# BUBLET/uav-airvision

Measured on AMD Instinct MI355X. Metric: stereo frames/sec (LK+stereo+MSCKF-update) at 752x480, higher is better.
Workload: dtype u8/int32 windows, f32 normal equations

## Files before the change

uav_airvision_amd/csrc/msckf.hip:

```cpp
#include <math.h>

#include <memory>
#include <new>
#include <vector>

#include "av_common.h"

namespace {

constexpr int IMU_DIM = 21;

#ifndef AV_FILTER_WAVE_PRIO
#define AV_FILTER_WAVE_PRIO 3
#endif
#define AV_FILTER_PRIO() __builtin_amdgcn_s_setprio(AV_FILTER_WAVE_PRIO)

__device__ __forceinline__ double av_rsqrt_f64(double d)
{
    const bool tiny = d < 1e-280;
    const double ds = tiny ? d * 0x1p200 : d;
    double y = __builtin_amdgcn_rsq(ds);
    const double h = 0.5 * ds;
    y = y * (1.5 - h * y * y);
    y = y * (1.5 - h * y * y);
// ... 772 lines not shown
        for (int r = 0; r < 3; ++r) sv[r] = u[r] / uu;
    } else if (tid == R2) {
        double dv[3] = {a.v_null[0] - a.v_new[0], a.v_null[1] - a.v_new[1], a.v_null[2] - a.v_new[2]};
        double dp[3] = {a.dt * a.v_null[0] + a.p_null[0] - a.p_new[0], a.dt * a.v_null[1] + a.p_null[1] - a.p_new[1], a.dt * a.v_null[2] + a.p_null[2] - a.p_new[2]};
        const double* g = a.gravity;
        w1[0] = -dv[2] * g[1] + dv[1] * g[2]; w1[1] = dv[2] * g[0] - dv[0] * g[2]; w1[2] = -dv[1] * g[0] + dv[0] * g[1];
        w2[0] = -dp[2] * g[1] + dp[1] * g[2]; w2[1] = dp[2] * g[0] - dp[0] * g[2]; w2[2] = -dp[1] * g[0] + dp[0] * g[1];
    }
    __syncthreads();
    __shared__ unsigned frow[IMU_DIM], fcol[IMU_DIM], prow[IMU_DIM];
    for (int i = tid; i < N * N; i += NT) F[i] *= a.dt;
    if (tid >= R2 && tid < R2 + N) {
        const int r = tid - R2; unsigned m = 0;
        for (int k = 0; k < N; ++k) if (F[r * N + k] != 0.0) m |= 1u << k;
        frow[r] = m;
    } else if (tid >= R3 && tid < R3 + N) {
        const int c = tid - R3; unsigned m = 0;
        for (int k = 0; k < N; ++k) if (F[k * N + c] != 0.0) m |= 1u << k;
        fcol[c] = m;
    }
    __syncthreads();
    for (int i = tid; i < N * N; i += NT) {
        int r = i / N, c = i - r * N; double s = 0;
        for (unsigned m = frow[r]; m; m &= m - 1) { const int k = __builtin_ctz(m); s += F[r * N + k] * F[k * N + c]; }
        F2[i] = s;
    }
    __syncthreads();
    for (int i = tid; i < N * N; i += NT) {
        int r = i / N, c = i - r * N; double s = 0;
        for (unsigned m = fcol[c]; m; m &= m - 1) { const int k = __builtin_ctz(m); s += F2[r * N + k] * F[k * N + c]; }
        Phi[i] = (r == c ? 1.0 : 0.0) + F[i] + F2[i] / 2. + s / 6.;
    }
    __syncthreads();
    if (tid < 9) {
        int r = tid / 3, c = tid % 3; double s = 0;
        for (int k = 0; k < 3; ++k) s += Rnew[r * 3 + k] * Rnull[c * 3 + k];
        Phi[r * N + c] = s;
    } else if (tid >= R1 && tid < R1 + 6) {
        const int t6 = tid - R1, blk = t6 / 3, r = t6 % 3;
        const int row = (blk == 0 ? 6 : 12) + r;
        const double* wv = blk == 0 ? w1 : w2;
        const double p0 = Phi[row * N], p1 = Phi[row * N + 1], p2 = Phi[row * N + 2];
        const double Au = p0 * u[0] + p1 * u[1] + p2 * u[2];
        const double d = Au - wv[r];
        Phi[row * N] = p0 - d * sv[0]; Phi[row * N + 1] = p1 - d * sv[1]; Phi[row * N + 2] = p2 - d * sv[2];
    } else if (tid >= R2 && tid < R2 + N) {
        const int r = tid - R2; unsigned m = 0;
        for (int k = 0; k < N; ++k) if (Phi[r * N + k] != 0.0) m |= 1u << k;
        if (r < 3 || (r >= 6 && r < 9) || (r >= 12 && r < 15)) m |= 7u;
        prow[r] = m;
    }
    __syncthreads();
    for (int i = tid; i < N * 12; i += NT) {
        int r = i / 12, c = i - r * 12; double s = 0;
        for (unsigned m = prow[r]; m; m &= m - 1) { const int k = __builtin_ctz(m); s += Phi[r * N + k] * G[k * 12 + c]; }
        T[i] = s;
    }
    for (int i = tid; i < N * N; i += NT) {
        int r = i / N, c = i - r * N; double s = 0;
        if (P11s) { for (unsigned m = prow[r]; m; m &= m - 1) { const int k = __builtin_ctz(m); s += Phi[r * N + k] * P11s[k * N + c]; } }
        else      { for (unsigned m = prow[r]; m; m &= m - 1) { const int k = __builtin_ctz(m); s += Phi[r * N + k] * a.P[(size_t)k * a.ld + c]; } }
        F2[i] = s;
        if (P11s) {
            double s2 = 0;
            for (unsigned m = prow[r]; m; m &= m - 1) { const int k = __builtin_ctz(m); s2 += Phi[r * N + k] * PhiT[k * N + c]; }
            Q[i] = s2;
        }
    }
    __syncthreads();
    for (int i = tid; i < N * N; i += NT) {
        int r = i / N, c = i - r * N; double s = 0, q = 0;
        for (int k = 0; k < 12; ++k) q += T[r * 12 + k] * a.noise[k / 3] * T[c * 12 + k];
        q = q * a.dt;
        for (unsigned m = prow[c]; m; m &= m - 1) { const int k = __builtin_ctz(m); s += F2[r * N + k] * Phi[c * N + k]; }
        F[i] = s + q;
    }
    __syncthreads();
    if (P11s) {
        for (int i = tid; i < N * N; i += NT) {
            int r = i / N, c = i - r * N;
            PhiT[i] = Q[i];
            P11s[i] = (F[r * N + c] + F[c * N + r]) / 2.;
        }
        __syncthreads();
        return;
    }
    const int nc = a.n - N;
    for (int c0 = 0; c0 < nc; c0 += N) {
        const int w = min(N, nc - c0);
        for (int i = tid; i < N * w; i += NT) {
            int r = i / w, c = i - r * w; double s = 0;
            for (unsigned m = prow[r]; m; m &= m - 1) { const int k = __builtin_ctz(m); s += Phi[r * N + k] * a.P[(size_t)k * a.ld + N + c0 + c]; }
            T[i] = s;
        }
        __syncthreads();
        for (int i = tid; i < N * w; i += NT) {
            int r = i / w, c = i - r * w;
            a.P[(size_t)r * a.ld + N + c0 + c] = T[i];
            a.P[(size_t)(N + c0 + c) * a.ld + r] = T[i];
        }
        __syncthreads();
    }
    for (int i = tid; i < N * N; i += NT) {
        int r = i / N, c = i - r * N;
        a.P[(size_t)r * a.ld + c] = (F[r * N + c] + F[c * N + r]) / 2.;
    }
}

__global__ __launch_bounds__(256) void propagate_kernel(PropArgs a) { propagate_body(a); }

struct AugArgs { double* P; int n, ld; double R_ic[9]; double sk[9]; };

template <int NT = 256>
__device__ __forceinline__ void augment_body(const AugArgs& a)
{
    __shared__ double J[6 * IMU_DIM];
    __shared__ double C[36];
    const int tid = threadIdx.x, N = IMU_DIM, n = a.n;
    for (int i = tid; i < 6 * N; i += NT) J[i] = 0.0;
    __syncthreads();
    if (tid < 9) {
        int r = tid / 3, c = tid % 3;
        J[r * N + c] = a.R_ic[tid];
        J[r * N + 15 + c] = r == c ? 1.0 : 0.0;
        J[(3 + r) * N + c] = a.sk[tid];
        J[(3 + r) * N + 12 + c] = r == c ? 1.0 : 0.0;
        J[(3 + r) * N + 18 + c] = r == c ? 1.0 : 0.0;
    }
    __syncthreads();
    for (int i = tid; i < 6 * n; i += NT) {
        int r = i / n, c = i - r * n; double s = 0;
        for (int k = 0; k < N; ++k) s += J[r * N + k] * a.P[(size_t)k * a.ld + c];
        a.P[(size_t)(n + r) * a.ld + c] = s;
    }
    __syncthreads();
    if (tid < 36) {
        int r = tid / 6, c = tid % 6; double s = 0;
        for (int k = 0; k < N; ++k) s += a.P[(size_t)(n + r) * a.ld + k] * J[c * N + k];
        C[tid] = s;
    }
    __syncthreads();
    for (int i = tid; i < 6 * n; i += NT) {
        int r = i / n, c = i - r * n;
        a.P[(size_t)c * a.ld + n + r] = a.P[(size_t)(n + r) * a.ld + c];
    }
    if (tid < 36) {
        int r = tid / 6, c = tid % 6;
        a.P[(size_t)(n + r) * a.ld + n + c] = (C[r * 6 + c] + C[c * 6 + r]) / 2.;
    }
}

__global__ __launch_bounds__(256) void augment_kernel(AugArgs a) { augment_body(a); }

__device__ __forceinline__ void remove_cam_body(double* P, double* scratch, int n, int ld, int start)
{
    const int tid = threadIdx.x, m = n - 6;
    for (int i = tid; i < m * m; i += (int)blockDim.x) {
        int r = i / m, c = i - r * m;
        int sr = r < start ? r : r + 6, sc = c < start ? c : c + 6;
        scratch[i] = P[(size_t)sr * ld + sc];
    }
    __syncthreads();
    for (int i = tid; i < m * m; i += (int)blockDim.x) {
        int r = i / m, c = i - r * m;
        P[(size_t)r * ld + c] = scratch[i];
    }
}
__device__ __forceinline__ void remove_two_cams_body(double* P, double* scratch, int n, int ld, int s0, int s1)
{
    const int tid = threadIdx.x, m = n - 12;
    for (int i = tid; i < m * m; i += (int)blockDim.x) {
        const int r = i / m, c = i - r * m;
        if (r < s0 && c < s0) continue;
        const int sr = r < s0 ? r : (r + 6 < s1 ? r + 6 : r + 12), sc = c < s0 ? c : (c + 6 < s1 ? c + 6 : c + 12);
        scratch[i] = P[(size_t)sr * ld + sc];
    }
    __syncthreads();
    for (int i = tid; i < m * m; i += (int)blockDim.x) {
        const int r = i / m, c = i - r * m;
        if (r < s0 && c < s0) continue;
        P[(size_t)r * ld + c] = scratch[i];
    }
}
__global__ __launch_bounds__(256) void remove_cam_kernel(double* P, double* scratch, int n, int ld, int start) { remove_cam_body(P, scratch, n, ld, start); }

struct UpdArgs {
    double* P; int n, ld;
    const double* Hsrc; const double* rsrc;
    const int* blk_row; const int* blk_len; int n_blk;
    double* W;
    int ldt;
    const int* cols; int nc;
    unsigned long long* prof;
    double* T;
    double* Kt;
    double* Pn;
    double* dx;
    double obs_noise;
    int m;
    double* Sbuf;
    int mode;
    int kdir;
    int round;
    int hld;
    int* status;
};
constexpr int UPD_BAD_PIVOT = -2;

template <typename T> using av_gptr = T __attribute__((address_space(1)))*;
struct UpdArgsG {
    av_gptr<double> P; int n, ld;
    av_gptr<const double> Hsrc; av_gptr<const double> rsrc;
    av_gptr<const int> blk_row; av_gptr<const int> blk_len; int n_blk;
    av_gptr<double> W; int ldt;
    av_gptr<const int> cols; int nc;
    av_gptr<unsigned long long> prof;
    av_gptr<double> T; av_gptr<double> Kt; av_gptr<double> Pn; av_gptr<double> dx;
    double obs_noise; int m;
    av_gptr<double> Sbuf;
    int mode, kdir, round, hld;
    av_gptr<int> status;
};
__device__ __forceinline__ UpdArgsG upd_load(const UpdArgs* __restrict__ arr, int i)
{
    const UpdArgs a = arr[i];
    UpdArgsG g;
    g.P = (av_gptr<double>)a.P; g.n = a.n; g.ld = a.ld; g.Hsrc = (av_gptr<const double>)a.Hsrc; g.rsrc = (av_gptr<const double>)a.rsrc;
    g.blk_row = (av_gptr<const int>)a.blk_row; g.blk_len = (av_gptr<const int>)a.blk_len; g.n_blk = a.n_blk;
    g.W = (av_gptr<double>)a.W; g.ldt = a.ldt; g.cols = (av_gptr<const int>)a.cols; g.nc = a.nc; g.prof = (av_gptr<unsigned long long>)a.prof;
    g.T = (av_gptr<double>)a.T; g.Kt = (av_gptr<double>)a.Kt; g.Pn = (av_gptr<double>)a.Pn; g.dx = (av_gptr<double>)a.dx;
    g.obs_noise = a.obs_noise; g.m = a.m; g.Sbuf = (av_gptr<double>)a.Sbuf; g.mode = a.mode; g.kdir = a.kdir; g.round = a.round; g.hld = a.hld;
    g.status = (av_gptr<int>)a.status;
    return g;
}

constexpr int UT = 1024;

__host__ __device__ inline bool upd_compress(int m, int nc) { return m > nc && (2 * m > 3 * nc || m > 136); }
__host__ __device__ inline int upd_k(int m, int nc) { return upd_compress(m, nc) ? nc : m; }

__device__ __forceinline__ double block_sum(double v, double* red)
{
    const int tid = threadIdx.x;
    v = wave_sum_f64(v);
    __syncthreads();
    if ((tid & 63) == 0) red[tid >> 6] = v;
    __syncthreads();
    double s = 0;
#pragma unroll
    for (int i = 0; i < UT / 64; ++i) s += red[i];
    return s;
}


__device__ __forceinline__ void reflector_scalars(double nrm2, double ajj, double& alpha, double& v0, double& tau)
{
    double r = nrm2 > 0 ? __builtin_amdgcn_rsq(nrm2) : 0.0;
    r = r * (1.5 - 0.5 * nrm2 * r * r);
    r = r * (1.5 - 0.5 * nrm2 * r * r);
    const double nrm = nrm2 * r;
    alpha = ajj >= 0 ? -nrm : nrm;
    v0 = ajj - alpha;
    const double vtv = nrm2 - 2 * alpha * ajj + alpha * alpha;
    double t = vtv > 0 ? __builtin_amdgcn_rcp(vtv) : 0.0;
    t = t * (2.0 - vtv * t);
    t = t * (2.0 - vtv * t);
    tau = 2.0 * t;
}

template <int CPW, int RPL>
__device__ __forceinline__ void qr_in_registers(const UpdArgs& a, int m, int nc, const int* srcrow, double* vb0, double* vb1, double* qsc,
                                                double* Wt, size_t ldt, double* rcol)
{
    const int tid = threadIdx.x, wave = tid >> 6, lane = tid & 63;
    double x[CPW][RPL];
#pragma unroll
    for (int l = 0; l < CPW; ++l) {
        const int c = wave + 16 * l;
#pragma unroll
        for (int t = 0; t < RPL; ++t) {
            const int row = lane + 64 * t;
            double v = 0.0;
            if (row < m && c <= nc) v = c < nc ? a.Hsrc[(size_t)srcrow[row] * a.ld + a.cols[c]] : a.rsrc[srcrow[row]];
            x[l][t] = v;
        }
    }
    __syncthreads();
    if (a.prof && tid == 0) a.prof[1] = __builtin_amdgcn_s_memrealtime();
    for (int j = 0; j < nc; ++j) {
        double* vb = (j & 1) ? vb1 : vb0;
        double* sc = qsc + 2 * (j & 1);
        if (wave == (j & 15)) {
            const int lj = j >> 4, tj = j >> 6;
            double part = 0, cand = 0;
#pragma unroll
            for (int l = 0; l < CPW; ++l) if (l == lj) {
#pragma unroll
                for (int t = 0; t < RPL; ++t) {
                    const int row = lane + 64 * t;
                    if (row >= j) part += x[l][t] * x[l][t];
                    if (t == tj) cand = x[l][t];
                }
            }
            const double nrm2 = wave_sum_f64(part);
            const double ajj = __shfl(cand, j & 63, 64);
            double alpha, v0o, tauo;
// ... 1053 lines not shown
```

uav_airvision_amd/csrc/msckf_dev.inc:

```

namespace {

constexpr int DEV_BUCKETS = 2;
constexpr int DEV_IMU_BATCH = 16;
constexpr int DEV_LDS_KEYS = 2048;

enum { DFAIL_NONE = 0, DFAIL_CAMS = 1, DFAIL_FRAMES = 2, DFAIL_STACK = 3, DFAIL_PIVOT = 4, DFAIL_TABLE = 5, DFAIL_OBS = 6, DFAIL_ROWS = 7 };

struct DState {
    double ts;
    double q[4], p[3], v[3], bg[3], ba[3];
    double R_ic[9], t_ci[3];
    double qn[4], pn[3], vn[3];
    double gravity[3];
    double tracking_rate;
    long long next_imu_id;
    int n, ncam;
    int active;
    int failed;
    int first_img, null_aliased;
    int prune, rm0, rm1;
    int n_prune_steps;
    int n_two_pass;
    int resets;
// ... 115 lines not shown
    for (int i = 0; i < 4; ++i) S.q[i] = qo[i];
    for (int i = 0; i < 3; ++i) {
        S.bg[i] += dx[3 + i]; S.v[i] += dx[6 + i]; S.ba[i] += dx[9 + i]; S.p[i] += dx[12 + i];
        if (S.null_aliased) { S.vn[i] += dx[6 + i]; S.pn[i] += dx[12 + i]; }
    }
    double de[4], Re[9], Rn[9];
    h_small_angle(dx + 15, de); h_to_rotation(de, Re);
    for (int r = 0; r < 3; ++r) for (int c = 0; c < 3; ++c) Rn[r * 3 + c] = Re[r * 3] * S.R_ic[c] + Re[r * 3 + 1] * S.R_ic[3 + c] + Re[r * 3 + 2] * S.R_ic[6 + c];
    for (int i = 0; i < 9; ++i) S.R_ic[i] = Rn[i];
    for (int i = 0; i < 3; ++i) S.t_ci[i] += dx[18 + i];
}
__device__ void dev_inject_cam(double* cq, double* cp, const double* d)
{
    double q4[4], co[4];
    h_small_angle(d, q4); h_quat_mul(q4, cq, co);
    for (int i = 0; i < 4; ++i) cq[i] = co[i];
    for (int i = 0; i < 3; ++i) cp[i] += d[3 + i];
}
__device__ void dev_apply_update(const DevArgs& a, int s, DState* D)
{
    const int st = a.stacked[s];
    if (threadIdx.x == 0) {
        if (st == UPD_BAD_PIVOT) D->failed = DFAIL_PIVOT;
        else if (st < 0) D->failed = DFAIL_STACK;
        else if (st > 0) { DState L = *D; dev_inject_imu(L, a.dx + (size_t)s * a.ld); *D = L; }
    }
    if (st > 0 && (int)threadIdx.x < D->ncam) {
        const size_t c = (size_t)s * a.cs + threadIdx.x;
        dev_inject_cam(a.cam_q + 4 * c, a.cam_p + 3 * c, a.dx + (size_t)s * a.ld + IMU_DIM + 6 * threadIdx.x);
    }
    __syncthreads();
}

__global__ __launch_bounds__(64) void dk_state(DevArgs a)
{
    AV_FILTER_PRIO();
    const int s = blockIdx.x * 64 + threadIdx.x;
    if (blockIdx.x == 0 && threadIdx.x < 16) a.cnt_next[threadIdx.x] = 0;
    if (s >= a.S) return;
    DState* Dg = a.st + s;
    const DCtl C = a.ctl[s];
    {
        DState L = *Dg;
        DState* D = &L;
        DCov cv; cv.act = 0; cv.cnt = 0; cv.first = C.imu_first; cv.pad = 0;
        if (C.has_init) {
            for (int i = 0; i < 4; ++i) D->q[i] = C.q0[i];
            for (int i = 0; i < 3; ++i) { D->bg[i] = C.bg0[i]; D->gravity[i] = C.g0[i]; }
        }
        int act = C.active && !D->failed;
        if (act && D->ncam + 1 > a.cs) { D->failed = DFAIL_CAMS; act = 0; }
        if (act && D->first_img) { D->first_img = 0; D->ts = C.t_frame; }
        D->active = act; D->prune = 0;
        if (act) {
            double* P = a.P + (size_t)s * a.pstride;
            const int n = D->n, ld = a.ld;
            for (int k = 0; k < C.imu_cnt; ++k) {
                PropArgs pa;
                const DImu m = a.imu[C.imu_first + k];
                pa.P = P; pa.n = n; pa.ld = ld; pa.dt = m.t - D->ts;
                for (int i = 0; i < 3; ++i) { pa.gyro[i] = m.w[i] - D->bg[i]; pa.acc[i] = m.a[i] - D->ba[i]; pa.gravity[i] = D->gravity[i]; }
                for (int i = 0; i < 4; ++i) { pa.q_old[i] = D->q[i]; pa.noise[i] = a.noise[i]; }
                dev_predict_new_state(*D, pa.dt, pa.gyro, pa.acc);
                for (int i = 0; i < 4; ++i) { pa.q_new[i] = D->q[i]; pa.q_null[i] = D->qn[i]; }
                for (int i = 0; i < 3; ++i) { pa.v_null[i] = D->vn[i]; pa.p_null[i] = D->pn[i]; pa.v_new[i] = D->v[i]; pa.p_new[i] = D->p[i]; }
                for (int i = 0; i < 4; ++i) D->qn[i] = D->q[i];
                for (int i = 0; i < 3; ++i) { D->pn[i] = D->p[i]; D->vn[i] = D->v[i]; }
                D->null_aliased = 1;
                D->ts = m.t;
                a.prop[C.imu_first + k] = pa;
            }
            double Rwi[9], Rwc[9], tw[3], cq[4];
            h_to_rotation(D->q, Rwi);
            for (int r = 0; r < 3; ++r) for (int c = 0; c < 3; ++c) Rwc[r * 3 + c] = D->R_ic[r * 3] * Rwi[c] + D->R_ic[r * 3 + 1] * Rwi[3 + c] + D->R_ic[r * 3 + 2] * Rwi[6 + c];
            h_mtv(Rwi, D->t_ci, tw);
            h_to_quaternion(Rwc, cq);
            const size_t c = (size_t)s * a.cs + D->ncam;
            a.cam_id[c] = D->next_imu_id++;
            for (int i = 0; i < 4; ++i) { a.cam_q[4 * c + i] = cq[i]; a.cam_qn[4 * c + i] = cq[i]; }
            for (int i = 0; i < 3; ++i) a.cam_p[3 * c + i] = D->p[i] + tw[i];
            cv.act = 1; cv.cnt = C.imu_cnt;
            cv.aa.P = P; cv.aa.n = n; cv.aa.ld = ld;
            for (int i = 0; i < 9; ++i) cv.aa.R_ic[i] = D->R_ic[i];
            const double sk[9] = {0, -tw[2], tw[1], tw[2], 0, -tw[0], -tw[1], tw[0], 0};
            for (int i = 0; i < 9; ++i) cv.aa.sk[i] = sk[i];
            D->n = n + 6; D->ncam += 1;
            a.ncam[s] = D->ncam; a.nstate[s] = D->n;
            for (int i = 0; i < 3; ++i) a.grav[3 * s + i] = D->gravity[i];
        }
        a.cov[s] = cv;
        *Dg = L;
    }
}

struct DImuState { double t, p[3], q[4], v[3], w[3]; };
static_assert(sizeof(DImuState) == 112, "av_imu_state is 112 bytes");
struct IrOut { DImuState* rec; int* n; int cap; };
__global__ __launch_bounds__(64) void dk_imu_rate(DevArgs a, IrOut R)
{
    AV_FILTER_PRIO();
    const int s = blockIdx.x, lane = threadIdx.x;
    const DCov cv = a.cov[s];
    const int had = cv.act ? cv.cnt : 0, wr = had < R.cap ? had : R.cap, k0 = had - wr;
    if (lane == 0) { R.n[2 * (size_t)s] = had; R.n[2 * (size_t)s + 1] = wr; }
    constexpr int W = (int)(sizeof(DImuState) / 8);
    double* out = reinterpret_cast<double*>(R.rec + (size_t)s * R.cap);
    for (int e = lane; e < wr * W; e += 64) {
        const int j = e / W, f = e - j * W;
        const size_t i = (size_t)cv.first + k0 + j;
        const PropArgs& pa = a.prop[i];
        out[e] = f == 0 ? a.imu[i].t : (f < 4 ? pa.p_new[f - 1] : (f < 8 ? pa.q_new[f - 4] : (f < 11 ? pa.v_new[f - 8] : pa.gyro[f - 11])));
    }
}

template <int NT>
__global__ __launch_bounds__(NT) void dk_cov(DevArgs a)
{
    AV_FILTER_PRIO();
    __shared__ double P11s[IMU_DIM * IMU_DIM], PhiT[IMU_DIM * IMU_DIM], work[PROP_LDS_DOUBLES];
    const int s = blockIdx.x, tid = threadIdx.x, N = IMU_DIM;
    const DCov cv = a.cov[s];
    if (!cv.act) return;
    double* P = cv.aa.P;
    const int n = cv.aa.n, ld = cv.aa.ld;
    auto stamp = [&](int i) { if (a.prof && s == 0 && tid == 0) a.prof[i] = __builtin_amdgcn_s_memrealtime(); };
    stamp(0);
    if (cv.cnt > 0) {
        for (int i = tid; i < N * N; i += NT) { const int r = i / N, c = i - r * N; P11s[i] = P[(size_t)r * ld + c]; PhiT[i] = r == c ? 1.0 : 0.0; }
        __syncthreads();
        for (int k = 0; k < cv.cnt; ++k) propagate_body<true, NT>(a.prop[cv.first + k], P11s, PhiT, work);
        stamp(1);
        const int nc = n - N;
        constexpr int CW = 64, NRQ = NT / CW;
        const int cl = tid % CW, rq = tid / CW;
        for (int c0 = 0; c0 < nc; c0 += CW) {
            const int c = c0 + cl;
            const bool in = c < nc;
            __syncthreads();
            for (int k = rq; k < IMU_DIM; k += NRQ) work[k * CW + cl] = in ? P[(size_t)k * ld + N + c] : 0.0;
            __syncthreads();
#pragma unroll 1
            for (int r = rq; r < IMU_DIM; r += NRQ) {
                double sum = 0;
#pragma unroll 7
                for (int k = 0; k < IMU_DIM; ++k) sum += PhiT[r * N + k] * work[k * CW + cl];
                if (in) { P[(size_t)r * ld + N + c] = sum; P[(size_t)(N + c) * ld + r] = sum; }
            }
        }
        for (int i = tid; i < N * N; i += NT) { const int r = i / N, c = i - r * N; P[(size_t)r * ld + c] = P11s[i]; }
        __syncthreads();
    }
    stamp(2);
    augment_body<NT>(cv.aa);
}

__device__ void dev_build_candidates(const DevArgs& a, const AvsTeam& T, const AvsStore& V, int s, int nc, const int* cand, bool full,
                                     int i0, int i1, const int* e0, const int* e1, int ph, int* lb )
{
    const int tid = threadIdx.x;
    const size_t f0 = (size_t)s * a.FS, ob = (size_t)s * a.obs_stride;
    if (tid < 8) lb[tid] = 0;
    __syncthreads();
    int obs_run = 0, row_run = 0, tobs_run = 0;
    for (int base = 0; base < nc; base += (int)blockDim.x) {
        const int k = base + tid;
        const bool in = k < nc;
        const int fs = in ? cand[k] : 0;
        const int nall = in ? V.m_nobs[fs] : 0;
        const int nobs = full ? nall : (in ? 2 : 0);
        const int init = in ? V.m_init[fs] : 1;
        int to, tr, tt;
        const int o = obs_run + T.excl_scan(nobs, &to);
        const int r = row_run + T.excl_scan(in ? 4 * nobs - 3 : 0, &tr);
        const int t = tobs_run + T.excl_scan((!full && !init) ? nall : 0, &tt);
        if (in) {
            const size_t f = f0 + k;
            a.f_off[f] = (int)(ob + o); a.f_rowoff[f] = r; a.f_dof[f] = full ? nobs - 1 : 2; a.f_mslot[f] = fs;
            if (!full) a.t_off[f] = (int)(ob + t);
            if (full) (void)avs_collect(V, fs, a.obs_cam + ob + o, a.obs_z + 4 * (ob + o));
            else {
                a.obs_cam[ob + o] = i0; a.obs_cam[ob + o + 1] = i1;
                const double* z0 = V.fr_z + ((size_t)avs_lslot(e0[k]) * V.cap + avs_lidx(e0[k])) * 4;
                const double* z1 = V.fr_z + ((size_t)avs_lslot(e1[k]) * V.cap + avs_lidx(e1[k])) * 4;
                for (int e = 0; e < 4; ++e) { a.obs_z[4 * (ob + o) + e] = z0[e]; a.obs_z[4 * (ob + o + 1) + e] = z1[e]; }
            }
            int valid = 1, tri = 0;
            if (init) { for (int e = 0; e < 3; ++e) a.f_pos[3 * f + e] = V.m_pos[(size_t)3 * fs + e]; }
            else {
                valid = 0; tri = 1;
                int* tc = full ? a.obs_cam + ob + o : a.t_obs_cam + ob + t;
                double* tz = full ? a.obs_z + 4 * (ob + o) : a.t_obs_z + 4 * (ob + t);
                if (!full) (void)avs_collect(V, fs, tc, tz);
                if (a.trans_thr >= 0) {
                    const size_t ca = (size_t)s * a.cs + tc[0], cb = (size_t)s * a.cs + tc[nall - 1];
                    double Ra[9], d[3] = {tz[0], tz[1], 1.0}, dw[3];
                    const double nd = h_norm3(d); d[0] /= nd; d[1] /= nd; d[2] /= nd;
                    h_to_rotation(a.cam_q + 4 * ca, Ra); h_mtv(Ra, d, dw);
                    const double tv[3] = {a.cam_p[3 * cb] - a.cam_p[3 * ca], a.cam_p[3 * cb + 1] - a.cam_p[3 * ca + 1], a.cam_p[3 * cb + 2] - a.cam_p[3 * ca + 2]};
                    const double par = tv[0] * dw[0] + tv[1] * dw[1] + tv[2] * dw[2];
                    const double o3[3] = {tv[0] - par * dw[0], tv[1] - par * dw[1], tv[2] - par * dw[2]};
                    if (!(h_norm3(o3) > a.trans_thr)) tri = 0;
                }
            }
            a.f_valid[f] = valid;
            const int bk = (full && nobs > 8) ? 1 : 0;
            V.tmp_a[k] = (bk << 24) | atomicAdd(&lb[bk], 1);
            V.tmp_b[k] = tri ? atomicAdd(&lb[5], 1) : -1;
        }
        obs_run += to; row_run += tr; tobs_run += tt;
    }
    __syncthreads();
    if (tid == 0) {
        a.f_off[f0 + nc] = (int)(ob + obs_run);
        if (!full) a.t_off[f0 + nc] = (int)(ob + tobs_run);
        a.n_cand[s] = nc;
        int shift = 0;
        if (row_run > a.rows_cap) {
            const int base = ph == 0 ? atomicAdd(&a.cnt[8 * ph + 4], row_run) : -1;
            if (base >= 0 && base + row_run <= a.pool_rows) shift = (a.S - s) * a.rows_cap + base;
            else shift = -1;
        }
        lb[6] = shift;
        a.over[s] = 0;
        if (shift < 0) { DState* D = a.st + s; D->failed = DFAIL_ROWS; D->active = 0; a.n_cand[s] = 0; }
    }
    __syncthreads();
    const int shift = lb[6];
    if (shift < 0) {
        for (int k = tid; k < nc; k += (int)blockDim.x) { a.f_rowoff[f0 + k] = -1; a.f_valid[f0 + k] = 0; V.tmp_b[k] = -1; }
        __syncthreads();
        return;
    }
    if (tid < 6) { const int c = lb[tid]; lb[tid] = c > 0 ? atomicAdd(&a.cnt[8 * ph + tid], c) : 0; }
    __syncthreads();
    const size_t lstride = (size_t)a.S * a.cap;
    for (int k = tid; k < nc; k += (int)blockDim.x) {
        const size_t f = f0 + k;
        const int v = V.tmp_a[k], bk = v >> 24;
        a.blist[bk * lstride + lb[bk] + (v & 0xFFFFFF)] = (int)f;
        if (V.tmp_b[k] >= 0) a.tlist[lb[5] + V.tmp_b[k]] = (int)f;
        if (shift > 0) a.f_rowoff[f] += shift;
    }
    __syncthreads();
}

__device__ __forceinline__ void dk_append_body(const DevArgs& a, unsigned long long* lds_keys)
{
    __shared__ int red[8], lb[8];
    const int s = blockIdx.x, tid = threadIdx.x;
    DState* D = a.st + s;
    if (!D->active) { if (tid == 0) { a.n_cand[s] = 0; a.over[s] = 0; a.f_off[(size_t)s * a.FS] = 0; } return; }
    AvsTeam T; T.red = red;
    AvsStore V = dev_store(a, s);
    if (a.cap <= DEV_LDS_KEYS) V.keys = lds_keys;
    const int before = V.hdr[AVS_LIVE];
    __syncthreads();
    auto stamp = [&](int i) { if (a.prof && s == 0 && tid == 0) a.prof[i] = __builtin_amdgcn_s_memrealtime(); };
    stamp(3);
    int tracked = 0;
    const int nk = a.msg_n[s] < a.msg_cap ? a.msg_n[s] : a.msg_cap;
    const int slot = avs_add_frame(T, V, a.msg_ids + (size_t)s * a.msg_cap, a.msg_uv + (size_t)s * a.msg_cap * 4, nk, &tracked);
    if (slot < 0) {
        if (tid == 0) { D->failed = slot == -1 ? DFAIL_FRAMES : DFAIL_TABLE; D->active = 0; a.n_cand[s] = 0; a.over[s] = 0; }
        return;
    }
    if (tid == 0) D->tracking_rate = tracked / ((double)before + 1e-5);
    int* cand = a.cand + (size_t)s * a.cap; int* inval = a.e0 + (size_t)s * a.cap;
    int nc = 0, ni = 0;
    stamp(4);
    avs_select_lost(T, V, cand, &nc, inval, &ni);
    stamp(5);
    dev_build_candidates(a, T, V, s, nc, cand, true, 0, 0, nullptr, nullptr, 0, lb);
    stamp(6);
    dev_triangulate_own(a, V, s, nc, false);
    stamp(7);
    if (tid == 0 && lb[6] > 0) D->n_two_pass += 1;
    avs_erase(T, V, cand, nc);
    avs_erase(T, V, inval, ni);
    stamp(8);
}

__device__ __forceinline__ void dk_begin_body(const DevArgs& a)
{
    AV_FILTER_PRIO();
    __shared__ unsigned long long keys8[DEV_LDS_KEYS];
    dk_append_body(a, keys8);
}
__global__ __launch_bounds__(256, 5) void dk_begin4(DevArgs a) { dk_begin_body(a); }

__device__ void dev_find_redundant(const DevArgs& a, int s, const DState& D, int* r0, int* r1)
{
    const int nc = D.ncam, key = nc - 4;
    const size_t c0 = (size_t)s * a.cs;
    int idx = key + 1, firstc = 0;
    double Rk[9];
    h_to_rotation(a.cam_q + 4 * (c0 + key), Rk);
    int sel[2];
    for (int k = 0; k < 2; ++k) {
        double Rc[9], RR[9], qq[4];
        h_to_rotation(a.cam_q + 4 * (c0 + idx), Rc);
        for (int r = 0; r < 3; ++r) for (int c = 0; c < 3; ++c) RR[r * 3 + c] = Rc[r * 3] * Rk[c * 3] + Rc[r * 3 + 1] * Rk[c * 3 + 1] + Rc[r * 3 + 2] * Rk[c * 3 + 2];
        h_to_quaternion(RR, qq);
        const double d[3] = {a.cam_p[3 * (c0 + idx)] - a.cam_p[3 * (c0 + key)], a.cam_p[3 * (c0 + idx) + 1] - a.cam_p[3 * (c0 + key) + 1], a.cam_p[3 * (c0 + idx) + 2] - a.cam_p[3 * (c0 + key) + 2]};
        const double ang = 2 * acos(qq[3]);
        if (ang < 0.2618 && h_norm3(d) < 0.4 && D.tracking_rate > 0.5) sel[k] = idx;
        else { sel[k] = firstc; ++firstc; }
// ... 542 lines not shown
```

Before: 233,000.

## Specialize covariance kernel for 64-thread blocks with sparsity-masked propagation chains

Adds a dk_cov<64> specialization that runs IMU covariance propagation, cross-covariance update and state augmentation with a single wavefront. It uses per-row and per-column nonzero bitmasks of F and Phi to skip zero terms in the matrix products, and keeps the working matrices in a compact LDS struct sized so the kernel can share a CU with the LK tracker. Cross and augment products are done per column in registers with explicit global address-space pointers. The risks are a mismatch in floating-point summation order, the extra complexity of the sparse indexing, and lower parallelism from using only 64 threads per block.

```diff
diff --git a/profiles/dk_cov_chains/summarise_traces.py b/profiles/dk_cov_chains/summarise_traces.py
--- /dev/null
+++ b/profiles/dk_cov_chains/summarise_traces.py
@@ -0,0 +1,51 @@
+#!/usr/bin/env python3
+import csv
+import glob
+import json
+import os
+import re
+import sys
+
+WATCH = ('dk_cov<64>', 'lk_track_g16_kernel<15>')
+
+
+def short(name):
+    name = re.sub(r'\(anonymous namespace\)::', '', name).replace('void ', '')
+    return re.sub(r'\(.*$', '', name)
+
+
+def stats(path):
+    rows = {}
+    for r in csv.DictReader(open(path)):
+        calls, mean = int(r['Calls']), float(r['AverageNs'])
+        rows[short(r['Name'])] = dict(calls=calls, mean_us=mean / 1e3, min_us=float(r.get('MinNs') or 'nan') / 1e3, max_us=float(r.get('MaxNs') or 'nan') / 1e3,
+                                      total_ms=float(r.get('TotalDurationNs') or calls * mean) / 1e6)
+    return rows
+
+
+def main():
+    out, summary = sys.argv[1], {}
+    for run in ('exclusive', 'shared'):
+        for tag in ('parent', 'this'):
+            found = glob.glob(os.path.join(out, 'trace_%s_%s' % (run, tag), '**', '*kernel_stats.csv'), recursive=True)
+            if not found:
+                continue
+            rows = stats(found[0])
+            line = open(os.path.join(out, 'bench_%s_traced_%s.jsonl' % (run, tag))).read().strip()
+            bench = json.loads(line) if line else {}
+            top = sorted(rows.items(), key=lambda kv: -kv[1]['total_ms'])[:10]
+            summary['%s_%s' % (run, tag)] = dict(watch={k: rows.get(k) for k in WATCH}, top10={k: v for k, v in top},
+                                                 value=bench.get('value'), kernel_ms_per_step=bench.get('kernel_ms_per_step'))
+            print('== %s, %s library: %s stereo frames/s under the tracer' % (run, tag, bench.get('value')))
+            for k in WATCH:
+                v = rows.get(k)
+                if v:
+                    print('  %-28s calls %5d  mean %9.1f us  min %9.1f  max %9.1f' % (k, v['calls'], v['mean_us'], v['min_us'], v['max_us']))
+            for k, v in top:
+                print('    top %-40s calls %5d  mean %9.1f us  total %9.2f ms' % (k[:40], v['calls'], v['mean_us'], v['total_ms']))
+            print('  kernel_ms_per_step %s' % json.dumps(bench.get('kernel_ms_per_step')))
+    json.dump(summary, open(os.path.join(out, 'trace_summary.json'), 'w'), indent=1, sort_keys=True)
+
+
+if __name__ == '__main__':
+    main()
diff --git a/uav_airvision_amd/csrc/msckf.hip b/uav_airvision_amd/csrc/msckf.hip
--- a/uav_airvision_amd/csrc/msckf.hip
+++ b/uav_airvision_amd/csrc/msckf.hip
@@ -948,6 +948,349 @@
 
 __global__ __launch_bounds__(256) void augment_kernel(AugArgs a) { augment_body(a); }
 
+constexpr int CVC_NN = IMU_DIM * IMU_DIM, CVC_NR = 9 * IMU_DIM;
+constexpr int CVC_PHIA = 0, CVC_PP = CVC_NN, CVC_FD = 2 * CVC_NN, CVC_F2 = CVC_FD + CVC_NR, CVC_PH = CVC_F2 + CVC_NR, CVC_PHIB = CVC_PH + CVC_NR,
+              CVC_P11 = CVC_PHIB + CVC_NN, CVC_DOUBLES = CVC_P11 + CVC_NN;
+struct CovChainsLds {
+    double m[CVC_DOUBLES];
+    double Rwi[9], Rnull[9], Rnew[9], u[3], sv[3], w1[3], w2[3];
+    unsigned frow[9], fcol[IMU_DIM], prow[9], pad;
+};
+static_assert(sizeof(CovChainsLds) <= 21760, "four of dk_cov<64>'s wavefronts beside twenty of LK's on a CU");
+static_assert(IMU_DIM * 12 <= 2 * CVC_NR && 2 * 6 * IMU_DIM + 36 <= CVC_NN, "T over Fdt | Fdt^2, the augmentation's matrices over Phi P11");
+using cvc_gptr = double __attribute__((address_space(1)))*;
+__device__ __forceinline__ cvc_gptr cvc_in_row(cvc_gptr row, unsigned bytes) { return (cvc_gptr)((char __attribute__((address_space(1)))*)row + bytes); }
+
+__device__ __forceinline__ int cvc_full(int q) { return q + 3 * (q / 3); }
+__device__ __forceinline__ int cvc_stored(int r) { return r - 3 * (r / 6); }
+__device__ __forceinline__ int cvc_unit_row(int u) { return u < 6 ? 3 + 6 * (u / 3) + u % 3 : 9 + u; }
+__device__ __forceinline__ double cvc_pick3(int i, double a0, double a1, double a2) { return i == 0 ? a0 : (i == 1 ? a1 : a2); }
+template <int n> __device__ __forceinline__ unsigned cvc_union(const unsigned* m)
+{
+    unsigned u = 0;
+#pragma unroll
+    for (int i = 0; i < n; ++i) u |= m[i];
+    return __builtin_amdgcn_readfirstlane(u);
+}
+__device__ __forceinline__ double cvc_G(const double* Rwi, int k, int c)
+{
+    const int b = k / 3;
+    const bool in = k < 12 && c / 3 == b;
+    double v = c == k ? (b == 0 ? -1.0 : 1.0) : 0.0;
+    if (b == 2) v = -Rwi[(in ? c - 6 : 0) * 3 + (k - 6)];
+    return in ? v : 0.0;
+}
+
+template <int J> __device__ __forceinline__ void cvc_noise(const double* T, const double* noise, const int (&r)[J], const int (&c)[J], double (&q)[J])
+{
+#pragma clang fp contract(off)
+#pragma unroll
+    for (int j = 0; j < J; ++j) q[j] = 0;
+#pragma unroll 1
+    for (int b = 0; b < 4; ++b) {
+        const double nz = noise[b];
+#pragma unroll 1
+        for (int kk = 0; kk < 3; ++kk) {
+            const int k = 3 * b + kk;
+            double x[J], y[J];
+#pragma unroll
+            for (int j = 0; j < J; ++j) { x[j] = T[r[j] * 12 + k]; y[j] = T[c[j] * 12 + k]; }
+#pragma unroll
+            for (int j = 0; j < J; ++j) q[j] = __builtin_fma(x[j] * nz, y[j], q[j]);
+        }
+    }
+}
+
+__device__ __forceinline__ void cvc_prepare(const PropArgs& a, CovChainsLds& L, int tid)
+{
+    const int N = IMU_DIM;
+    double* const F = L.m + CVC_FD;
+    for (int i = tid; i < CVC_NR; i += 64) F[i] = 0.0;
+    if (tid < 3) quat_to_rot(tid == 0 ? a.q_old : (tid == 1 ? a.q_null : a.q_new), tid == 0 ? L.Rwi : (tid == 1 ? L.Rnull : L.Rnew));
+    __syncthreads();
+    if (tid < 9) {
+        const int r = tid / 3, c = tid - 3 * r;
+        const double* w = a.gyro; const double* ac = a.acc;
+        const double* Rwi = L.Rwi;
+        const double skw = cvc_pick3(r, cvc_pick3(c, 0.0, -w[2], w[1]), cvc_pick3(c, w[2], 0.0, -w[0]), cvc_pick3(c, -w[1], w[0], 0.0));
+        F[r * N + c] = -skw;
+        F[r * N + 3 + c] = r == c ? -1.0 : 0.0;
+        double s = __builtin_fma(Rwi[r], cvc_pick3(c, 0.0, -ac[2], ac[1]), 0.0);
+        s = __builtin_fma(Rwi[3 + r], cvc_pick3(c, ac[2], 0.0, -ac[0]), s);
+        s = __builtin_fma(Rwi[6 + r], cvc_pick3(c, -ac[1], ac[0], 0.0), s);
+        F[(3 + r) * N + c] = -s;
+        F[(3 + r) * N + 9 + c] = -Rwi[c * 3 + r];
+        F[(6 + r) * N + 6 + c] = r == c ? 1.0 : 0.0;
+    } else if (tid == 9) {
+        const double* Rnull = L.Rnull; double* u = L.u; double* sv = L.sv;
+        for (int r = 0; r < 3; ++r) u[r] = Rnull[r * 3] * a.gravity[0] + Rnull[r * 3 + 1] * a.gravity[1] + Rnull[r * 3 + 2] * a.gravity[2];
+        double uu = u[0] * u[0] + u[1] * u[1] + u[2] * u[2];
+        for (int r = 0; r < 3; ++r) sv[r] = u[r] / uu;
+    } else if (tid == 22) {
+        double* w1 = L.w1; double* w2 = L.w2;
+        double dv[3] = {a.v_null[0] - a.v_new[0], a.v_null[1] - a.v_new[1], a.v_null[2] - a.v_new[2]};
+        double dp[3] = {a.dt * a.v_null[0] + a.p_null[0] - a.p_new[0], a.dt * a.v_null[1] + a.p_null[1] - a.p_new[1], a.dt * a.v_null[2] + a.p_null[2] - a.p_new[2]};
+        const double* g = a.gravity;
+        w1[0] = -dv[2] * g[1] + dv[1] * g[2]; w1[1] = dv[2] * g[0] - dv[0] * g[2]; w1[2] = -dv[1] * g[0] + dv[0] * g[1];
+        w2[0] = -dp[2] * g[1] + dp[1] * g[2]; w2[1] = dp[2] * g[0] - dp[0] * g[2]; w2[2] = -dp[1] * g[0] + dp[0] * g[1];
+    }
+    __syncthreads();
+}
+
+__device__ __forceinline__ void cvc_patch(CovChainsLds& L, int tid)
+{
+    const int N = IMU_DIM;
+    double* const Phi = L.m + CVC_PH;
+    if (tid < 9) {
+        const double* Rnew = L.Rnew; const double* Rnull = L.Rnull;
+        int r = tid / 3, c = tid % 3; double s = 0;
+        for (int k = 0; k < 3; ++k) s += Rnew[r * 3 + k] * Rnull[c * 3 + k];
+        Phi[r * N + c] = s;
+    } else if (tid >= 9 && tid < 9 + 6) {
+        const double* u = L.u; const double* sv = L.sv;
+        const int t6 = tid - 9, blk = t6 / 3, r = t6 % 3;
+        const int row = (blk == 0 ? 3 : 6) + r;
+        const double* wv = blk == 0 ? L.w1 : L.w2;
+        const double p0 = Phi[row * N], p1 = Phi[row * N + 1], p2 = Phi[row * N + 2];
+        const double Au = p0 * u[0] + p1 * u[1] + p2 * u[2];
+        const double d = Au - wv[r];
+        Phi[row * N] = p0 - d * sv[0]; Phi[row * N + 1] = p1 - d * sv[1]; Phi[row * N + 2] = p2 - d * sv[2];
+    } else if (tid >= 22 && tid < 22 + 9) {
+        const int q = tid - 22; unsigned m = 0;
+        for (int k = 0; k < N; ++k) if (Phi[q * N + k] != 0.0) m |= 1u << k;
+        L.prow[q] = m | 7u;
+    }
+    __syncthreads();
+}
+
+__device__ __forceinline__ void propagate_chains(const PropArgs& a, CovChainsLds& L, const double* PhiT, double* PhiTn)
+{
+#pragma clang fp contract(off)
+    int tid = threadIdx.x;
+    asm volatile("" : "+v"(tid));
+    const int N = IMU_DIM;
+    double* const F = L.m + CVC_FD, * const F2 = L.m + CVC_F2, * const Phi = L.m + CVC_PH, * const T = L.m + CVC_FD, * const PP = L.m + CVC_PP,
+          * const P11 = L.m + CVC_P11;
+    constexpr unsigned STORED = 0x71C7u;
+    const double dt = a.dt;
+    cvc_prepare(a, L, tid);
+    for (int i = tid; i < CVC_NR; i += 64) F[i] *= dt;
+    __syncthreads();
+    if (tid >= 22 && tid < 22 + 9) {
+        const int q = tid - 22; unsigned m = 0;
+        for (int k = 0; k < N; ++k) if (F[q * N + k] != 0.0) m |= 1u << k;
+        L.frow[q] = m & STORED;
+    } else if (tid >= 43) {
+        const int c = tid - 43; unsigned m = 0;
+        for (int q = 0; q < 9; ++q) if (F[q * N + c] != 0.0) m |= 1u << cvc_full(q);
+        L.fcol[c] = m;
+    }
+    __syncthreads();
+    int eq[3], ec[3]; bool eok[3];
+#pragma unroll
+    for (int j = 0; j < 3; ++j) { const int e = tid + 64 * j; eok[j] = e < CVC_NR; const int ee = eok[j] ? e : 0; eq[j] = ee / N; ec[j] = ee - eq[j] * N; }
+    {
+        unsigned m[3]; double s[3];
+#pragma unroll
+        for (int j = 0; j < 3; ++j) { m[j] = eok[j] ? L.frow[eq[j]] : 0u; s[j] = 0; }
+        for (unsigned U = cvc_union<9>(L.frow); U; U &= U - 1) {
+            const int k = __builtin_ctz(U), kq = cvc_stored(k);
+            double x[3], y[3];
+#pragma unroll
+            for (int j = 0; j < 3; ++j) { x[j] = F[eq[j] * N + k]; y[j] = F[kq * N + ec[j]]; }
+#pragma unroll
+            for (int j = 0; j < 3; ++j) if ((m[j] >> k) & 1u) s[j] = __builtin_fma(x[j], y[j], s[j]);
+        }
+#pragma unroll
+        for (int j = 0; j < 3; ++j) if (eok[j]) F2[tid + 64 * j] = s[j];
+    }
+    __syncthreads();
+    {
+        unsigned m[3]; double s[3];
+#pragma unroll
+        for (int j = 0; j < 3; ++j) { m[j] = eok[j] ? L.fcol[ec[j]] : 0u; s[j] = 0; }
+        for (unsigned U = cvc_union<IMU_DIM>(L.fcol); U; U &= U - 1) {
+            const int k = __builtin_ctz(U), kq = cvc_stored(k);
+            double x[3], y[3];
+#pragma unroll
+            for (int j = 0; j < 3; ++j) { x[j] = F2[eq[j] * N + k]; y[j] = F[kq * N + ec[j]]; }
+#pragma unroll
+            for (int j = 0; j < 3; ++j) if ((m[j] >> k) & 1u) s[j] = __builtin_fma(x[j], y[j], s[j]);
+        }
+#pragma unroll
+        for (int j = 0; j < 3; ++j) if (eok[j]) {
+            const int i = tid + 64 * j;
+            Phi[i] = __builtin_fma(F2[i], 0.5, (cvc_full(eq[j]) == ec[j] ? 1.0 : 0.0) + F[i]) + s[j] / 6.;
+        }
+    }
+    __syncthreads();
+    cvc_patch(L, tid);
+    {
+        int tq[2], tc[2]; bool tok[2]; unsigned m[3], mt[2]; double sp[3], sq[3], st[2];
+#pragma unroll
+        for (int j = 0; j < 3; ++j) { m[j] = eok[j] ? L.prow[eq[j]] : 0u; sp[j] = 0; sq[j] = 0; }
+#pragma unroll
+        for (int j = 0; j < 2; ++j) {
+            const int e = tid + 64 * j; tok[j] = e < 9 * 12; const int ee = tok[j] ? e : 0; tq[j] = ee / 12; tc[j] = ee - tq[j] * 12;
+            mt[j] = tok[j] ? L.prow[tq[j]] : 0u; st[j] = 0;
+        }
+        for (unsigned U = cvc_union<9>(L.prow); U; U &= U - 1) {
+            const int k = __builtin_ctz(U);
+            double x[3], p[3], f[3], xt[2], g[2];
+#pragma unroll
+            for (int j = 0; j < 3; ++j) { x[j] = Phi[eq[j] * N + k]; p[j] = P11[k * N + ec[j]]; f[j] = PhiT[k * N + ec[j]]; }
+#pragma unroll
+            for (int j = 0; j < 2; ++j) { xt[j] = Phi[tq[j] * N + k]; g[j] = cvc_G(L.Rwi, k, tc[j]); }
+#pragma unroll
+            for (int j = 0; j < 3; ++j) if ((m[j] >> k) & 1u) { sp[j] = __builtin_fma(x[j], p[j], sp[j]); sq[j] = __builtin_fma(x[j], f[j], sq[j]); }
+#pragma unroll
+            for (int j = 0; j < 2; ++j) if ((mt[j] >> k) & 1u) st[j] = __builtin_fma(xt[j], g[j], st[j]);
+        }
+#pragma unroll
+        for (int j = 0; j < 3; ++j) if (eok[j]) { const int i = cvc_full(eq[j]) * N + ec[j]; PP[i] = sp[j]; PhiTn[i] = sq[j]; }
+#pragma unroll
+        for (int j = 0; j < 2; ++j) if (tok[j]) T[cvc_full(tq[j]) * 12 + tc[j]] = st[j];
+#pragma unroll
+        for (int j = 0; j < 4; ++j) {
+            const int e = tid + 64 * j;
+            if (e < 12 * N) {
+                const int u = e / N, c = e - u * N, i = cvc_unit_row(u) * N + c;
+                PP[i] = __builtin_fma(1.0, P11[i], 0.0); PhiTn[i] = __builtin_fma(1.0, PhiT[i], 0.0);
+            }
+        }
+#pragma unroll
+        for (int j = 0; j < 3; ++j) {
+            const int e = tid + 64 * j;
+            if (e < 12 * 12) { const int u = e / 12, c = e - u * 12, r = cvc_unit_row(u); T[r * 12 + c] = r == c ? 1.0 : 0.0; }
+        }
+    }
+    __syncthreads();
+    {
+        int r[3], c[3], cq[3]; bool ok[3]; unsigned m[3]; double q[3], s[3];
+#pragma unroll
+        for (int j = 0; j < 3; ++j) {
+            const int e = tid + 64 * j; ok[j] = e < CVC_NR; const int ee = ok[j] ? e : 0; r[j] = ee / 9; cq[j] = ee - r[j] * 9; c[j] = cvc_full(cq[j]);
+            m[j] = ok[j] ? L.prow[cq[j]] : 0u; s[j] = 0;
+        }
+        cvc_noise<3>(T, a.noise, r, c, q);
+        for (unsigned U = cvc_union<9>(L.prow); U; U &= U - 1) {
+            const int k = __builtin_ctz(U);
+            double x[3], y[3];
+#pragma unroll
+            for (int j = 0; j < 3; ++j) { x[j] = PP[r[j] * N + k]; y[j] = Phi[cq[j] * N + k]; }
+#pragma unroll
+            for (int j = 0; j < 3; ++j) if ((m[j] >> k) & 1u) s[j] = __builtin_fma(x[j], y[j], s[j]);
+        }
+#pragma unroll
+        for (int j = 0; j < 3; ++j) if (ok[j]) P11[r[j] * N + c[j]] = __builtin_fma(q[j], dt, s[j]);
+    }
+    {
+        int r[4], c[4]; bool ok[4]; double q[4];
+#pragma unroll
+        for (int j = 0; j < 4; ++j) { const int e = tid + 64 * j; ok[j] = e < 12 * N; const int ee = ok[j] ? e : 0; r[j] = ee / 12; c[j] = cvc_unit_row(ee - r[j] * 12); }
+        cvc_noise<4>(T, a.noise, r, c, q);
+#pragma unroll
+        for (int j = 0; j < 4; ++j) if (ok[j]) { const int i = r[j] * N + c[j]; P11[i] = __builtin_fma(q[j], dt, __builtin_fma(PP[i], 1.0, 0.0)); }
+    }
+    __syncthreads();
+#pragma unroll
+    for (int j = 0; j < 7; ++j) {
+        const int i = tid + 64 * j, r = i / N, c = i - r * N;
+        if (i < CVC_NN && r <= c) { const double v = (P11[r * N + c] + P11[c * N + r]) / 2.; P11[r * N + c] = v; P11[c * N + r] = v; }
+    }
+    __syncthreads();
+}
+
+__device__ __forceinline__ void cross_chains(cvc_gptr P, int n, int ld, const double* PhiT)
+{
+#pragma clang fp contract(off)
+    int tid = threadIdx.x;
+    asm volatile("" : "+v"(tid));
+    const int N = IMU_DIM, nc = n - N;
+    for (int c0 = 0; c0 < nc; c0 += 64) {
+        const int c = c0 + tid;
+        if (c < nc) {
+            double w[IMU_DIM];
+            const unsigned cb = 8u * (unsigned)c;
+            const cvc_gptr mir = P + (size_t)(N + c) * ld;
+#pragma unroll
+            for (int k = 0; k < N; ++k) w[k] = *cvc_in_row(P + (size_t)k * ld + N, cb);
+#pragma unroll 1
+            for (int r = 0; r < N; r += 3) {
+                const double* ph = PhiT + r * N;
+                double s0 = 0, s1 = 0, s2 = 0;
+#pragma unroll
+                for (int k = 0; k < N; ++k) {
+                    s0 = __builtin_fma(ph[k], w[k], s0); s1 = __builtin_fma(ph[N + k], w[k], s1); s2 = __builtin_fma(ph[2 * N + k], w[k], s2);
+                    if (k % 3 == 2) __builtin_amdgcn_sched_barrier(0);
+                }
+                *cvc_in_row(P + (size_t)r * ld + N, cb) = s0; *cvc_in_row(P + (size_t)(r + 1) * ld + N, cb) = s1; *cvc_in_row(P + (size_t)(r + 2) * ld + N, cb) = s2;
+                mir[r] = s0; mir[r + 1] = s1; mir[r + 2] = s2;
+            }
+        }
+    }
+}
+
+__device__ __forceinline__ void augment_chains(const AugArgs& a, double* J, double* JP, double* C)
+{
+#pragma clang fp contract(off)
+    int tid = threadIdx.x;
+    asm volatile("" : "+v"(tid));
+    const int N = IMU_DIM, n = a.n, ld = a.ld;
+    const cvc_gptr P = (cvc_gptr)a.P;
+    for (int i = tid; i < 6 * N; i += 64) J[i] = 0.0;
+    __syncthreads();
+    if (tid < 9) {
+        int r = tid / 3, c = tid % 3;
+        J[r * N + c] = a.R_ic[tid];
+        J[r * N + 15 + c] = r == c ? 1.0 : 0.0;
+        J[(3 + r) * N + c] = a.sk[tid];
+        J[(3 + r) * N + 12 + c] = r == c ? 1.0 : 0.0;
+        J[(3 + r) * N + 18 + c] = r == c ? 1.0 : 0.0;
+    }
+    __syncthreads();
+#pragma unroll 1
+    for (int h = 0; h < 6; h += 3)
+    for (int c0 = 0; c0 < n; c0 += 64) {
+        const int c = c0 + tid;
+        if (c < n) {
+            double p[IMU_DIM], s[3];
+            int o = h * N;
+            asm volatile("" : "+s"(o));
+            const double* Jr = J + o;
+            const unsigned cb = 8u * (unsigned)c;
+            const cvc_gptr mir = P + (size_t)c * ld + n + h;
+#pragma unroll
+            for (int k = 0; k < N; ++k) p[k] = *cvc_in_row(P + (size_t)k * ld, cb);
+#pragma unroll
+            for (int r = 0; r < 3; ++r) s[r] = 0;
+#pragma unroll
+            for (int k = 0; k < N; ++k) {
+#pragma unroll
+                for (int r = 0; r < 3; ++r) s[r] = __builtin_fma(Jr[r * N + k], p[k], s[r]);
+                if (k % 3 == 2) __builtin_amdgcn_sched_barrier(0);
+            }
+#pragma unroll
+            for (int r = 0; r < 3; ++r) {
+                *cvc_in_row(P + (size_t)(n + h + r) * ld, cb) = s[r]; mir[r] = s[r];
+                if (c < N) JP[(h + r) * N + c] = s[r];
+            }
+        }
+    }
+    __syncthreads();
+    if (tid < 36) {
+        int r = tid / 6, c = tid % 6; double s = 0;
+#pragma unroll
+        for (int k = 0; k < N; ++k) s = __builtin_fma(JP[r * N + k], J[c * N + k], s);
+        C[tid] = s;
+    }
+    __syncthreads();
+    if (tid < 36) {
+        int r = tid / 6, c = tid % 6;
+        P[(size_t)(n + r) * ld + n + c] = (C[r * 6 + c] + C[c * 6 + r]) / 2.;
+    }
+}
+
 __device__ __forceinline__ void remove_cam_body(double* P, double* scratch, int n, int ld, int start)
 {
     const int tid = threadIdx.x, m = n - 6;
diff --git a/uav_airvision_amd/csrc/msckf_dev.inc b/uav_airvision_amd/csrc/msckf_dev.inc
--- a/uav_airvision_amd/csrc/msckf_dev.inc
+++ b/uav_airvision_amd/csrc/msckf_dev.inc
@@ -291,6 +291,34 @@
     }
     stamp(2);
     augment_body<NT>(cv.aa);
+}
+template <>
+__global__ __launch_bounds__(256, 5) void dk_cov<64>(DevArgs a)
+{
+    AV_FILTER_PRIO();
+    __shared__ CovChainsLds L;
+    const int s = blockIdx.x, tid = threadIdx.x, N = IMU_DIM;
+    const DCov& cv = a.cov[s];
+    if (!cv.act) return;
+    const cvc_gptr P = (cvc_gptr)cv.aa.P;
+    const int n = cv.aa.n, ld = cv.aa.ld, cnt = cv.cnt, first = cv.first;
+    auto stamp = [&](int i) { if (a.prof && s == 0 && tid == 0) a.prof[i] = __builtin_amdgcn_s_memrealtime(); };
+    stamp(0);
+    if (cnt > 0) {
+        double* PhiT = L.m + CVC_PHIA, * PhiTn = L.m + CVC_PHIB, * const P11s = L.m + CVC_P11;
+        for (int i = tid; i < N * N; i += 64) { const int r = i / N, c = i - r * N; P11s[i] = P[(size_t)r * ld + c]; PhiT[i] = r == c ? 1.0 : 0.0; }
+        __syncthreads();
+        for (int k = 0; k < cnt; ++k) {
+            propagate_chains(a.prop[first + k], L, PhiT, PhiTn);
+            double* const t = PhiT; PhiT = PhiTn; PhiTn = t;
+        }
+        stamp(1);
+        cross_chains(P, n, ld, PhiT);
+        for (int i = tid; i < N * N; i += 64) { const int r = i / N, c = i - r * N; P[(size_t)r * ld + c] = P11s[i]; }
+        __syncthreads();
+    }
+    stamp(2);
+    augment_chains(cv.aa, L.m + CVC_PP, L.m + CVC_PP + 6 * N, L.m + CVC_PP + 12 * N);
 }
 
 __device__ void dev_build_candidates(const DevArgs& a, const AvsTeam& T, const AvsStore& V, int s, int nc, const int* cand, bool full,
```

Result: faster. 236,000 (median of 6 runs) (+1.3%).
